# sjtuytc/UnboundedNeRFPytorch

Hardware: AMD Instinct MI355X
Metric: Msamples/sec (Mip-360 garden-shaped 1920x1080x256 frame, FourierGrid render) (higher is better)
Workload: dtype f32; 1 GPU; S1 1920x1080x256 G200 F3(P7) C12 rgbnet 39-128-128-3 f32 stepsize 1.31 thres 1e-4 white-noise grids; rays=2073600, samples_per_ray=256, chunks_per_frame=1, parallelism=1 GPU, step=ray generation + march + shade + un-tiling to image order; 3 frames in flight

## Files before the change

### unboundednerfpytorch_amd/csrc/ugrid_march.hip

```cpp
#include "ugrid_render.h"
#include "ugrid_rays.h"
#include "ugrid_tensorf.h"

__global__ void k_pack_bricks(const float *__restrict__ grid, int P, int C, int X, int Y, int Z, int H,
                              int CH, int coef, float *__restrict__ out, int64_t total) {
  for (int64_t o = (int64_t)blockIdx.x * blockDim.x + threadIdx.x; o < total;
       o += (int64_t)gridDim.x * blockDim.x) {
    int64_t q = o;
    int ch, c;
    if (H == 2) {
      const int qi = (int)(q % (8 * CH)); q /= (8 * CH);
      c = (qi >> 1) & 7;
      ch = (qi >> 4) * 2 + (qi & 1);
    } else {
      ch = (int)(q % CH); q /= CH;
      c = (int)(q % 8); q /= 8;
    }
    const int h = (int)(q % H); q /= H;
    const int k = (int)(q % (Z - 1)); q /= (Z - 1);
    const int j = (int)(q % (Y - 1)); q /= (Y - 1);
    const int i = (int)(q % (X - 1)); q /= (X - 1);
    const int l = (int)q;
    const int chan = h * CH + ch;
    float v = 0.f;
// ... 905 lines not shown
  if (n_rays <= 0) return 0;
  if (n_steps < 2 || !act_shift || mpi_depth < 1 || mpi_depth > 256 || !scratch_w || !scratch_T || !count2 || !alphainv_last)
    return (int)hipErrorInvalidValue;
  ug_train_vox v;
  const int rc = ug_fill_train_vox(&v, mask, mask_dims3, xyz2ijk_scale3, xyz2ijk_shift3);
  if (rc) return rc;
  v.plane_shift = act_shift; v.D = mpi_depth;
  ug_train_args a;
  a.n_rays = n_rays; a.S = n_steps; a.P = 1; a.F = 0; a.X = X; a.Y = Y; a.Z = Z; a.norm_l2 = 0;
  a.cx = a.cy = a.cz = 0.f; a.rx = a.ry = a.rz = 1.f; a.B = 1.f; a.A = 0.f;
  a.shift = 0.f; a.interval = interval; a.thres = thres;
  hipLaunchKernelGGL(HIP_KERNEL_NAME(k_train_march_vox<3>), dim3(ug_blocks(n_rays * UG_WAVE, 256)), dim3(256), 0, ST(s), a, v, density_grid,
                     rays_o, rays_d, (const float *)nullptr, xyz_min, xyz_max, scratch_pts, scratch_density, scratch_step, count, scratch_w,
                     scratch_T, count2, alphainv_last);
  UG_LAUNCH_CHECK();
  return 0;
}

extern "C" int ugrid_train_sample_compact_vox(int64_t n_rays, int32_t slots_per_ray, float act_shift, float interval, float thres,
                                              const float *scratch_pts, const float *scratch_density, const int32_t *scratch_step,
                                              const float *scratch_w, const float *scratch_T, const int32_t *count,
                                              const int64_t *offset_end, const int32_t *count2, const int64_t *offset_end2,
                                              const float *t_table, float *pts1, float *density1, float *weights1, float *T1,
                                              int32_t *pos2, float *pts2, float *density2, float *alpha2, float *weights2,
                                              int64_t *ray_id2, int64_t *step_id2, float *t2, uint8_t *inner2, ugrid_stream_t s) {
  if (n_rays <= 0) return 0;
  hipLaunchKernelGGL(k_train_compact2, dim3(ug_blocks(n_rays * UG_WAVE, 256)), dim3(256), 0, ST(s), n_rays, slots_per_ray, act_shift,
                     interval, thres, scratch_pts, scratch_density, scratch_step, scratch_w, scratch_T, count, offset_end, count2,
                     offset_end2, t_table, pts1, density1, weights1, T1, pos2, pts2, density2, alpha2, weights2, ray_id2, step_id2, t2,
                     inner2, ug_tl_devn.cap > 0 ? ug_tl_devn.cap : INT64_MAX);
  UG_LAUNCH_CHECK();
  return 0;
}

extern "C" int ugrid_train_sample_backward(int64_t n_rays, float act_shift, float interval, const float *density1,
                                           const float *weights1, const float *T1, const int32_t *pos2, const int32_t *count,
                                           const int64_t *offset_end, const float *alphainv_last, const float *g_weights2,
                                           const float *g_alphainv_last, const float *g_density2, float *g_density1,
                                           ugrid_stream_t s) {
  if (n_rays <= 0) return 0;
  hipLaunchKernelGGL(k_train_sample_bwd, dim3(ug_blocks(n_rays * UG_WAVE, 256)), dim3(256), 0, ST(s), n_rays, act_shift, interval,
                     density1, weights1, T1, pos2, count, offset_end, alphainv_last, g_weights2, g_alphainv_last, g_density2, g_density1);
  UG_LAUNCH_CHECK();
  return 0;
}

extern "C" int ugrid_train_compact(int64_t n_rays, int32_t n_samples, const float *scratch_pts, const float *scratch_density,
                                   const int32_t *scratch_step, const int32_t *count, const int64_t *offset_end,
                                   const float *t_table, float *pts, float *density, int64_t *ray_id, int64_t *step_id,
                                   float *t, ugrid_stream_t s) {
  if (n_rays <= 0) return 0;
  hipLaunchKernelGGL(k_train_compact, dim3(ug_blocks(n_rays * UG_WAVE, 256)), dim3(256), 0, ST(s), n_rays, n_samples,
                     scratch_pts, scratch_density, scratch_step, count, offset_end, t_table, pts, density, ray_id, step_id, t);
  UG_LAUNCH_CHECK();
  return 0;
}

template <class MarchTile>
__device__ __forceinline__ void ug_march_block(const ug_ws_view &ws, int64_t nblocks, MarchTile march) {
  const int64_t blk = ug_xcd_remap(blockIdx.x, nblocks);
  if (blk >= nblocks) return;
  const int64_t tile = blk * 4 + (threadIdx.x >> 6);
  if (tile >= ws.n_tiles) return;
  const int n = march(tile, ws.ent + tile * ws.cap, ws.slot + tile * ws.cap);
  if (ug_lane() == 0) ws.count[tile] = n;
}

struct ug_march_geom { ug_ws_view ws; int64_t nblocks; dim3 grid; };
static inline ug_march_geom ug_march_geometry(void *ws_mem, int64_t n_rays, int32_t S) {
  ug_march_geom g;
  g.ws = ug_ws_make(ws_mem, n_rays, S);
  g.nblocks = (g.ws.n_tiles + 3) / 4;
  g.grid = dim3((unsigned)(((g.nblocks + 7) / 8) * 8));
  return g;
}

template <int F, bool L2, int W>
__global__ void __launch_bounds__(256, W)
k_march(ug_march_args a, const float *__restrict__ rays_o, const float *__restrict__ rays_d,
        const float *__restrict__ t_table, const float *__restrict__ s_table,
        const float *__restrict__ bricks, float *__restrict__ alphainv_last, float *__restrict__ depth,
        ug_ws_view ws, int64_t nblocks) {
  ug_march_block(ws, nblocks, [&](int64_t tile, float4 *ent, uint8_t *slot) {
    return ug_march_tile<F, L2>(a, rays_o, rays_d, t_table, s_table, bricks, alphainv_last, depth, tile, ent, slot);
  });
}


template <bool L2>
__global__ void __launch_bounds__(256, 5)
k_march_dcvgo(ug_march_args a, ug_dc_args dc, const float *__restrict__ rays_o, const float *__restrict__ rays_d,
              const float *__restrict__ t_table, const float *__restrict__ s_table, const float *__restrict__ bricks,
              float *__restrict__ alphainv_last, float *__restrict__ depth, float *__restrict__ wsum_mid, ug_ws_view ws,
              int64_t nblocks) {
  ug_march_block(ws, nblocks, [&](int64_t tile, float4 *ent, uint8_t *slot) {
    return ug_march_tile<0, L2, true>(a, rays_o, rays_d, t_table, s_table, bricks, alphainv_last, depth, tile, ent, slot, dc, wsum_mid);
  });
}

__global__ void __launch_bounds__(256, 6)
k_march_dvgo(ug_march_args a, ug_dv_args dv, const float *__restrict__ rays_o, const float *__restrict__ rays_d,
             const float *__restrict__ bricks, float *__restrict__ alphainv_last, float *__restrict__ depth, ug_ws_view ws,
             int64_t nblocks) {
  ug_march_block(ws, nblocks, [&](int64_t tile, float4 *ent, uint8_t *slot) {
    return ug_march_tile_dvgo(a, dv, rays_o, rays_d, bricks, alphainv_last, depth, tile, ent, slot, a.S);
  });
}

__global__ void __launch_bounds__(256, 6)
k_march_mpi(ug_march_args a, ug_mpi_args mp, const float *__restrict__ rays_o, const float *__restrict__ rays_d,
            const float *__restrict__ bricks, const float *__restrict__ act_shift, float *__restrict__ alphainv_last,
            float *__restrict__ depth, ug_ws_view ws, int64_t nblocks) {
  __shared__ float shift[256];
  if ((int)threadIdx.x < mp.D) shift[threadIdx.x] = act_shift[threadIdx.x];
  __syncthreads();
  ug_march_block(ws, nblocks, [&](int64_t tile, float4 *ent, uint8_t *slot) {
    return ug_march_tile_mpi(a, mp, rays_o, rays_d, bricks, shift, alphainv_last, depth, tile, ent, slot);
  });
}

extern "C" int64_t ugrid_render_ws_bytes(int64_t n_rays, int32_t S) {
  const int64_t n_tiles = (n_rays + UG_WAVE - 1) / UG_WAVE, cap = (int64_t)UG_WAVE * S;
  return 256 + ug_align256(n_tiles * 4) + ug_align256(n_tiles * cap * 16) + ug_align256(n_tiles * cap);
}

static int ug_grid_query_any(bool cl, const float *grid, int P, int C, int X, int Y, int Z, const float *xyz,
                             const float *xyz_min, const float *xyz_max, int freq_num, int64_t n, float *out, hipStream_t st) {
  if (n <= 0) return 0;
  if (P != (freq_num > 0 ? 2 * freq_num + 1 : 1)) return (int)hipErrorInvalidValue;
  const int64_t nl = ug_launch_rows(n);
  if (cl)
    hipLaunchKernelGGL(HIP_KERNEL_NAME(k_grid_query<true>), dim3(ug_blocks(nl * C, 256)), dim3(256), 0, st, grid, P, C, X, Y, Z, xyz,
                       xyz_min, xyz_max, freq_num, n, out, ug_tl_devn.ptr);
  else
    hipLaunchKernelGGL(HIP_KERNEL_NAME(k_grid_query<false>), dim3(ug_blocks(nl, 256)), dim3(256), 0, st, grid, P, C, X, Y, Z, xyz,
                       xyz_min, xyz_max, freq_num, n, out, ug_tl_devn.ptr);
  UG_LAUNCH_CHECK();
  return 0;
}

extern "C" int ugrid_grid_query(const float *grid, int P, int C, int X, int Y, int Z, const float *xyz,
                                const float *xyz_min, const float *xyz_max, int freq_num, int64_t n,
                                float *out, ugrid_stream_t s) {
  return ug_grid_query_any(false, grid, P, C, X, Y, Z, xyz, xyz_min, xyz_max, freq_num, n, out, ST(s));
}

extern "C" int ugrid_grid_query_cl(const float *grid, int P, int C, int X, int Y, int Z, const float *xyz,
                                   const float *xyz_min, const float *xyz_max, int freq_num, int64_t n,
                                   float *out, ugrid_stream_t s) {
  return ug_grid_query_any(true, grid, P, C, X, Y, Z, xyz, xyz_min, xyz_max, freq_num, n, out, ST(s));
}

static int ug_grid_query_backward_any(bool cl, const float *grad_out, int P, int C, int X, int Y, int Z, const float *xyz,
                                      const float *xyz_min, const float *xyz_max, int freq_num, int64_t n,
                                      float *grad_grid, hipStream_t st, uint32_t *touch = nullptr) {
  if (n <= 0) return 0;
  if (P != (freq_num > 0 ? 2 * freq_num + 1 : 1)) return (int)hipErrorInvalidValue;
  const int64_t nl = ug_launch_rows(n);
  if (cl)
    hipLaunchKernelGGL(HIP_KERNEL_NAME(k_grid_query_backward<true>), dim3(ug_blocks(nl * P * C, 256)), dim3(256), 0, st, grad_out, P, C,
                       X, Y, Z, xyz, xyz_min, xyz_max, freq_num, n, grad_grid, touch, ug_tl_devn.ptr);
  else
    hipLaunchKernelGGL(HIP_KERNEL_NAME(k_grid_query_backward<false>), dim3(ug_blocks(nl * P, 256)), dim3(256), 0, st, grad_out, P, C,
                       X, Y, Z, xyz, xyz_min, xyz_max, freq_num, n, grad_grid, (uint32_t *)nullptr, ug_tl_devn.ptr);
  UG_LAUNCH_CHECK();
  return 0;
}

extern "C" int ugrid_grid_query_backward(const float *grad_out, int P, int C, int X, int Y, int Z, const float *xyz,
                                         const float *xyz_min, const float *xyz_max, int freq_num, int64_t n,
                                         float *grad_grid, ugrid_stream_t s) {
  return ug_grid_query_backward_any(false, grad_out, P, C, X, Y, Z, xyz, xyz_min, xyz_max, freq_num, n, grad_grid, ST(s));
}

extern "C" int ugrid_grid_query_backward_cl(const float *grad_out, int P, int C, int X, int Y, int Z, const float *xyz,
                                            const float *xyz_min, const float *xyz_max, int freq_num, int64_t n,
                                            float *grad_grid, ugrid_stream_t s) {
  return ug_grid_query_backward_any(true, grad_out, P, C, X, Y, Z, xyz, xyz_min, xyz_max, freq_num, n, grad_grid, ST(s));
}

extern "C" int ugrid_grid_query_backward_cl_touch(const float *grad_out, int P, int C, int X, int Y, int Z, const float *xyz,
                                                  const float *xyz_min, const float *xyz_max, int freq_num, int64_t n,
                                                  float *grad_grid, uint32_t *touch, ugrid_stream_t s) {
  return ug_grid_query_backward_any(true, grad_out, P, C, X, Y, Z, xyz, xyz_min, xyz_max, freq_num, n, grad_grid, ST(s), touch);
}

extern "C" int ugrid_count_views_accumulate(const float *rays_o, const float *rays_d, int64_t n_rays, const float *xyz_min,
                                            const float *xyz_max, float near, float far, float stepdist, int32_t n_samples, int X, int Y,
                                            int Z, float *acc, ugrid_stream_t s) {
  if (n_rays <= 0 || n_samples <= 0) return 0;
  if (!rays_o || !rays_d || !xyz_min || !xyz_max || !acc || X < 1 || Y < 1 || Z < 1) return (int)hipErrorInvalidValue;
  hipLaunchKernelGGL(k_count_views_accumulate, dim3(ug_blocks(n_rays, 64)), dim3(64), 0, ST(s), rays_o, rays_d, n_rays, xyz_min, xyz_max,
                     near, far, stepdist, n_samples, X, Y, Z, acc);
  UG_LAUNCH_CHECK();
  return 0;
}

extern "C" int ugrid_count_views_commit(float *acc, float *count, int64_t n, ugrid_stream_t s) {
  if (n <= 0) return 0;
  if (!acc || !count) return (int)hipErrorInvalidValue;
  const int64_t blocks = ug_blocks(n, 256);
  hipLaunchKernelGGL(k_count_views_commit, dim3((unsigned)(blocks < 65536 ? blocks : 65536)), dim3(256), 0, ST(s), acc, count, n);
  UG_LAUNCH_CHECK();
  return 0;
}

static inline int ug_brick_ch(int C, int *H) {
  if (C == 1) { *H = 1; return 1; }
  *H = 2;
  return UG_CH(C);
}

extern "C" int64_t ugrid_brick_bytes(int P, int C, int X, int Y, int Z, int direct) {
  int H, CH = ug_brick_ch(C, &H);
  if (direct) { H = 1; CH = 4; }
  return (int64_t)P * (X - 1) * (Y - 1) * (Z - 1) * H * 8 * CH * (int64_t)sizeof(float);
}

extern "C" int ugrid_pack_bricks(const float *grid, int P, int C, int X, int Y, int Z, int direct,
                                 float *bricks, ugrid_stream_t s) {
  if (X < 2 || Y < 2 || Z < 2 || P < 1 || C < 1) return (int)hipErrorInvalidValue;
  int H, CH = ug_brick_ch(C, &H);
  if (direct) { H = 1; CH = 4; }
  const int64_t total = (int64_t)P * (X - 1) * (Y - 1) * (Z - 1) * H * 8 * CH;
  int64_t blocks = (total + 255) / 256;
  if (blocks > 256 * 64) blocks = 256 * 64;
  if (C == 12 && !direct) {
    if (P > 1 && (int64_t)(X - 1) * (Y - 1) * (Z - 1) * 384 >= ((int64_t)1 << 32)) return (int)hipErrorInvalidValue;
    hipLaunchKernelGGL(k_pack_quad, dim3((unsigned)blocks), dim3(256), 0, ST(s), grid, P, C, X, Y, Z, bricks, total);
    UG_LAUNCH_CHECK();
    return 0;
  }
  int coef = direct ? 0 : 1;
  hipLaunchKernelGGL(k_pack_bricks, dim3((unsigned)blocks), dim3(256), 0, ST(s), grid, P, C, X, Y, Z, H, CH,
                     coef, bricks, total);
  UG_LAUNCH_CHECK();
  return 0;
}

static int g_march_waves = 6;
extern "C" int ug_set_march_waves(int w) { if (w < 4 || w > 6) return 1; g_march_waves = w; return 0; }

template <int F, int W>
static int ug_march_launch_w(const ugrid_render_params *p, const ug_march_args &a, const float *rays_o,
                             const float *rays_d, const float *t_table, const float *s_table,
                             const float *bricks, float *alphainv_last, float *depth, const ug_march_geom &g,
                             hipStream_t st) {
  if (p->norm_l2)
    hipLaunchKernelGGL(HIP_KERNEL_NAME(k_march<F, true, W>), g.grid, dim3(256), 0, st, a, rays_o,
                       rays_d, t_table, s_table, bricks, alphainv_last, depth, g.ws, g.nblocks);
  else
    hipLaunchKernelGGL(HIP_KERNEL_NAME(k_march<F, false, W>), g.grid, dim3(256), 0, st, a, rays_o,
                       rays_d, t_table, s_table, bricks, alphainv_last, depth, g.ws, g.nblocks);
  UG_LAUNCH_CHECK();
  return 0;
}

template <int F>
static int ug_march_launch(const ugrid_render_params *p, const ug_march_args &a, const float *rays_o,
                           const float *rays_d, const float *t_table, const float *s_table,
                           const float *bricks, float *alphainv_last, float *depth, const ug_march_geom &g,
                           hipStream_t st) {
  switch (g_march_waves) {
    case 4: return ug_march_launch_w<F, 4>(p, a, rays_o, rays_d, t_table, s_table, bricks, alphainv_last, depth, g, st);
    case 6: return ug_march_launch_w<F, 6>(p, a, rays_o, rays_d, t_table, s_table, bricks, alphainv_last, depth, g, st);
    default: return ug_march_launch_w<F, 5>(p, a, rays_o, rays_d, t_table, s_table, bricks, alphainv_last, depth, g, st);
  }
}

extern "C" int ugrid_render_march(const ugrid_render_params *p, const float *rays_o, const float *rays_d,
                                  const float *t_table, const float *s_table, const float *density_bricks,
                                  float *alphainv_last, float *depth, void *ws_mem, ugrid_stream_t s) {
  if (p->n_rays <= 0) return 0;
  ug_march_args a;
  const int rc = ug_fill_march_args(p, a);
  if (rc) return rc;
  const ug_march_geom g = ug_march_geometry(ws_mem, p->n_rays, p->n_samples);
  switch (p->freq_num) {
    case 1: return ug_march_launch<1>(p, a, rays_o, rays_d, t_table, s_table, density_bricks, alphainv_last, depth, g, ST(s));
    case 2: return ug_march_launch<2>(p, a, rays_o, rays_d, t_table, s_table, density_bricks, alphainv_last, depth, g, ST(s));
    case 3: return ug_march_launch<3>(p, a, rays_o, rays_d, t_table, s_table, density_bricks, alphainv_last, depth, g, ST(s));
    case 4: return ug_march_launch<4>(p, a, rays_o, rays_d, t_table, s_table, density_bricks, alphainv_last, depth, g, ST(s));
    case 5: return ug_march_launch<5>(p, a, rays_o, rays_d, t_table, s_table, density_bricks, alphainv_last, depth, g, ST(s));
    default: return (int)hipErrorInvalidValue;
  }
}


extern "C" int ugrid_render_march_dcvgo(const ugrid_render_params *p, const ugrid_dcvgo_params *q, const float *rays_o,
                                        const float *rays_d, const float *t_table, const float *s_table,
                                        const float *density_bricks, float *alphainv_last, float *depth, float *wsum_mid,
                                        void *ws_mem, ugrid_stream_t s) {
  if (p->n_rays <= 0) return 0;
  if (p->freq_num != 0 || !q) return (int)hipErrorInvalidValue;
  ug_march_args a;
  ug_dc_args dc;
  int rc = ug_fill_mask_args(dc, q->mask, q->mask_x, q->mask_y, q->mask_z, q->xyz2ijk_scale, q->xyz2ijk_shift);
  if (!rc) rc = ug_fill_march_args(p, a);
  if (rc) return rc;
  dc.dist_thres = q->dist_thres;
  const ug_march_geom g = ug_march_geometry(ws_mem, p->n_rays, p->n_samples);
  if (p->norm_l2)
    hipLaunchKernelGGL(HIP_KERNEL_NAME(k_march_dcvgo<true>), g.grid, dim3(256), 0, ST(s), a, dc, rays_o, rays_d, t_table,
                       s_table, density_bricks, alphainv_last, depth, wsum_mid, g.ws, g.nblocks);
  else
    hipLaunchKernelGGL(HIP_KERNEL_NAME(k_march_dcvgo<false>), g.grid, dim3(256), 0, ST(s), a, dc, rays_o, rays_d, t_table,
                       s_table, density_bricks, alphainv_last, depth, wsum_mid, g.ws, g.nblocks);
  UG_LAUNCH_CHECK();
  return 0;
}


extern "C" int ugrid_render_march_dvgo(const ugrid_render_params *p, const ugrid_dvgo_params *q, const float *rays_o,
                                       const float *rays_d, const float *density_bricks, float *alphainv_last, float *depth,
                                       void *ws_mem, ugrid_stream_t s) {
  if (p->n_rays <= 0) return 0;
  if (p->freq_num != 0 || !q || !(q->stepdist > 0.f)) return (int)hipErrorInvalidValue;
  ug_march_args a;
  ug_dv_args dv;
  int rc = ug_fill_mask_args(dv, q->mask, q->mask_x, q->mask_y, q->mask_z, q->xyz2ijk_scale, q->xyz2ijk_shift);
  if (!rc) rc = ug_fill_march_args(p, a);
  if (rc) return rc;
  dv.near = q->near_clip; dv.far = q->far_clip; dv.stepdist = q->stepdist;
  const ug_march_geom g = ug_march_geometry(ws_mem, p->n_rays, p->n_samples);
  hipLaunchKernelGGL(k_march_dvgo, g.grid, dim3(256), 0, ST(s), a, dv, rays_o, rays_d, density_bricks, alphainv_last,
                     depth, g.ws, g.nblocks);
  UG_LAUNCH_CHECK();
  return 0;
}



extern "C" int ugrid_render_march_mpi(const ugrid_render_params *p, const ugrid_mpi_params *q, const float *rays_o,
                                      const float *rays_d, const float *density_bricks, const float *act_shift, float *alphainv_last,
                                      float *depth, void *ws_mem, ugrid_stream_t s) {
  if (p->n_rays <= 0) return 0;
  if (p->freq_num != 0 || !q || !act_shift) return (int)hipErrorInvalidValue;
  if (q->mpi_depth < 2 || q->mpi_depth > 256 || q->n_steps < 2 || q->n_steps > p->n_samples) return (int)hipErrorInvalidValue;
  ug_march_args a;
  ug_mpi_args mp;
  int rc = ug_fill_mask_args(mp, q->mask, q->mask_x, q->mask_y, q->mask_z, q->xyz2ijk_scale, q->xyz2ijk_shift);
  if (!rc) rc = ug_fill_march_args(p, a);
  if (rc) return rc;
  mp.D = q->mpi_depth; mp.n = q->n_steps;
  const ug_march_geom g = ug_march_geometry(ws_mem, p->n_rays, p->n_samples);
  hipLaunchKernelGGL(k_march_mpi, g.grid, dim3(256), 0, ST(s), a, mp, rays_o, rays_d, density_bricks, act_shift,
                     alphainv_last, depth, g.ws, g.nblocks);
  UG_LAUNCH_CHECK();
// ... 3 lines not shown
```

### unboundednerfpytorch_amd/csrc/ugrid_render.h

```cpp
#pragma once
#include "ugrid_common.h"
#include "ugrid_math.h"
#include <string.h>

#define UG_CH(C) (2 * (((C) + 3) / 4))
#define UG_MAX_F 5


typedef float f32x16 __attribute__((ext_vector_type(16)));

struct ug_vec3 { float x, y, z; };

__device__ __forceinline__ float ug_norm3_torch(float x, float y, float z) {
  return sqrtf(fmaf(z, z, fmaf(y, y, x * x)));
}

template <bool L2>
__device__ __forceinline__ ug_vec3 ug_contract(ug_vec3 p, float B, float A) {
  const float nrm = L2 ? ug_norm3_torch(p.x, p.y, p.z) : fmaxf(fabsf(p.x), fmaxf(fabsf(p.y), fabsf(p.z)));
  if (!(nrm <= 1.0f)) {
    const float sc = B - (1.0f / nrm) * A;
    p.x = p.x / nrm * sc;
    p.y = p.y / nrm * sc;
    p.z = p.z / nrm * sc;
// ... 20 lines not shown
    a.cell = i0; a.wlo = wlo; a.whi = whi;
  }
  return a;
}

struct ug_cellw { int64_t rec; float w[8]; };

__device__ __forceinline__ ug_cellw ug_cell_setup(float ux, float uy, float uz, int X, int Y, int Z,
                                                 int64_t level_base) {
  const ug_axis ax = ug_axis_setup(ux, X), ay = ug_axis_setup(uy, Y), az = ug_axis_setup(uz, Z);
  ug_cellw r;
  r.rec = level_base + ((int64_t)ax.cell * (Y - 1) + ay.cell) * (Z - 1) + az.cell;
  r.w[0] = az.wlo * ay.wlo * ax.wlo;
  r.w[1] = az.whi * ay.wlo * ax.wlo;
  r.w[2] = az.wlo * ay.whi * ax.wlo;
  r.w[3] = az.whi * ay.whi * ax.wlo;
  r.w[4] = az.wlo * ay.wlo * ax.whi;
  r.w[5] = az.whi * ay.wlo * ax.whi;
  r.w[6] = az.wlo * ay.whi * ax.whi;
  r.w[7] = az.whi * ay.whi * ax.whi;
  return r;
}

template <int F>
struct ug_levels { float cx[2 * F + 1], cy[2 * F + 1], cz[2 * F + 1]; };

template <int F>
__device__ __forceinline__ ug_levels<F> ug_pe(float ux, float uy, float uz) {
  ug_levels<F> L;
  L.cx[0] = ux; L.cy[0] = uy; L.cz[0] = uz;
#pragma unroll
  for (int k = 0; k < F; ++k) {
    const float f = (float)(1 << k);
    float s, c;
    sincosf(f * ux, &s, &c); L.cx[2 * k + 1] = s; L.cx[2 * k + 2] = c;
    sincosf(f * uy, &s, &c); L.cy[2 * k + 1] = s; L.cy[2 * k + 2] = c;
    sincosf(f * uz, &s, &c); L.cz[2 * k + 1] = s; L.cz[2 * k + 2] = c;
  }
  return L;
}

__device__ __forceinline__ float ug_unorm(float p, float lo, float hi) {
  return ((p - lo) / (hi - lo)) * 2.f - 1.f;
}

struct ug_ws_view {
  int32_t *count;
  float4 *ent;
  uint8_t *slot;
  int64_t n_tiles, cap;
};
#define UG_FEAT_STRIDE 12

__host__ __device__ static inline int64_t ug_align256(int64_t x) { return (x + 255) & ~(int64_t)255; }

static inline ug_ws_view ug_ws_make(void *ws, int64_t n_rays, int32_t S) {
  ug_ws_view v;
  v.n_tiles = (n_rays + UG_WAVE - 1) / UG_WAVE;
  v.cap = (int64_t)UG_WAVE * S;
  char *b = (char *)ws + 256;
  v.count = (int32_t *)b;
  b += ug_align256(v.n_tiles * (int64_t)sizeof(int32_t));
  v.ent = (float4 *)b;
  b += ug_align256(v.n_tiles * v.cap * (int64_t)sizeof(float4));
  v.slot = (uint8_t *)b;
  return v;
}

__device__ __forceinline__ int64_t ug_xcd_remap(int64_t b, int64_t nblocks) {
  const int64_t per = (nblocks + 7) / 8;
  return (b % 8) * per + b / 8;
}

struct ug_march_args {
  int64_t n_rays;
  int32_t S, X, Y, Z;
  float cx, cy, cz, rx, ry, rz;
  float lox, loy, loz, hix, hiy, hiz;
  float ex, ey, ez, irx, iry, irz;
  float B, A;
  float shift, interval, thres;
};

__device__ __forceinline__ float ug_density_level(const char *__restrict__ lvl, float cx, float cy, float cz,
                                                  int X, int Y, int Z) {
  const ug_axis_fast ax = ug_axis_inrange(cx, X), ay = ug_axis_inrange(cy, Y), az = ug_axis_inrange(cz, Z);
  const unsigned row = (unsigned)fmaf(ax.cellf, (float)(Y - 1), ay.cellf);
  const unsigned off = __umul24(row, (unsigned)(Z - 1) << 5) + ((unsigned)az.cell << 5);
  const float4 *b = (const float4 *)(lvl + off);
  const float4 v0 = b[0], v1 = b[1];
  const float tz = az.whi, ty = ay.whi, tx = ax.whi;
  const float p00 = fmaf(v0.y, tz, v0.x), p01 = fmaf(v0.w, tz, v0.z);
  const float p10 = fmaf(v1.y, tz, v1.x), p11 = fmaf(v1.w, tz, v1.z);
  return fmaf(fmaf(p11, ty, p10), tx, fmaf(p01, ty, p00));
}

__device__ __forceinline__ void ug_normalise(const ug_march_args &a, float px, float py, float pz, float &ux, float &uy, float &uz) {
  ux = ug_div_r(px - a.lox, a.ex, a.irx) * 2.f - 1.f;
  uy = ug_div_r(py - a.loy, a.ey, a.iry) * 2.f - 1.f;
  uz = ug_div_r(pz - a.loz, a.ez, a.irz) * 2.f - 1.f;
}

__device__ __forceinline__ bool ug_outside_box(const ug_march_args &a, float px, float py, float pz) {
  return (a.lox > px) | (a.loy > py) | (a.loz > pz) | (a.hix < px) | (a.hiy < py) | (a.hiz < pz);
}

struct ug_mask_args {
  const uint8_t *mask;
  int32_t mi, mj, mk;
  float sx, sy, sz, hx, hy, hz;
};

__device__ __forceinline__ bool ug_mask_lookup(const ug_mask_args &m, float px, float py, float pz) {
  float fi = roundf(px * m.sx + m.hx), fj = roundf(py * m.sy + m.hy), fk = roundf(pz * m.sz + m.hz);
  fi = (fi != fi) ? 0.f : fi; fj = (fj != fj) ? 0.f : fj; fk = (fk != fk) ? 0.f : fk;
  if (fi >= 0.f && fi < (float)m.mi && fj >= 0.f && fj < (float)m.mj && fk >= 0.f && fk < (float)m.mk)
    return m.mask[((int64_t)fi * m.mj + (int64_t)fj) * m.mk + (int64_t)fk] != 0;
  return false;
}

static inline int ug_fill_mask_args(ug_mask_args &m, const uint8_t *mask, int32_t mask_x, int32_t mask_y, int32_t mask_z,
                                    const float *scale3, const float *shift3) {
  if (!mask || !scale3 || !shift3 || mask_x < 1 || mask_y < 1 || mask_z < 1) return (int)hipErrorInvalidValue;
  m.mask = mask; m.mi = mask_x; m.mj = mask_y; m.mk = mask_z;
  m.sx = scale3[0]; m.sy = scale3[1]; m.sz = scale3[2];
  m.hx = shift3[0]; m.hy = shift3[1]; m.hz = shift3[2];
  return 0;
}

__device__ __forceinline__ bool ug_composite(float alpha, float thres, float &T, float &w, bool &done) {
  if (!(alpha > thres)) return false;
  w = T * alpha;
  T = (float)((double)T * (1. - (double)alpha));
  if ((double)T < 1e-3) done = true;
  return w > thres;
}

__device__ __forceinline__ void ug_append_survivors(bool surv, float px, float py, float pz, float w, int lane,
                                                    float4 *__restrict__ ent, uint8_t *__restrict__ slot, int &nsurv) {
  const unsigned long long m = __ballot(surv);
  if (m != 0ull) {
    if (surv) {
      const int idx = nsurv + __builtin_amdgcn_mbcnt_hi((unsigned)(m >> 32), __builtin_amdgcn_mbcnt_lo((unsigned)m, 0u));
      ent[idx] = make_float4(px, py, pz, w);
      slot[idx] = (uint8_t)lane;
    }
    nsurv += __popcll(m);
  }
}

struct ug_dc_args : ug_mask_args {
  float dist_thres;
};

template <int F, bool L2, bool DC = false>
__device__ __forceinline__ int ug_march_tile(const ug_march_args &a, const float *__restrict__ rays_o,
                                             const float *__restrict__ rays_d, const float *__restrict__ t_table,
                                             const float *__restrict__ s_table, const float *__restrict__ bricks,
                                             float *__restrict__ alphainv_last, float *__restrict__ depth,
                                             int64_t tile, float4 *__restrict__ ent, uint8_t *__restrict__ slot,
                                             const ug_dc_args &dc = ug_dc_args{}, float *__restrict__ wsum_mid = nullptr) {
  constexpr int P = 2 * F + 1;
  const int lane = ug_lane();
  const int64_t ray = tile * UG_WAVE + lane;
  const bool valid = ray < a.n_rays;

  float ox = 0.f, oy = 0.f, oz = 0.f, dx = 0.f, dy = 0.f, dz = 1.f;
  if (valid) {
    const float rox = rays_o[3 * ray], roy = rays_o[3 * ray + 1], roz = rays_o[3 * ray + 2];
    const float rdx = rays_d[3 * ray], rdy = rays_d[3 * ray + 1], rdz = rays_d[3 * ray + 2];
    ox = (rox - a.cx) / a.rx; oy = (roy - a.cy) / a.ry; oz = (roz - a.cz) / a.rz;
    const float dn = ug_norm3_torch(rdx, rdy, rdz);
    dx = rdx / dn; dy = rdy / dn; dz = rdz / dn;
  }

  const size_t lvl_bytes = (size_t)(a.X - 1) * (a.Y - 1) * (a.Z - 1) * 32;
  const char *__restrict__ bkb = (const char *)bricks;

  float T = 1.f, dsum = 0.f;
  bool done = !valid;
  int nsurv = 0;
  [[maybe_unused]] float cum = 0.f, ppx = 0.f, ppy = 0.f, ppz = 0.f, wmid = 0.f;

  for (int j = 0; j < a.S; ++j) {
    if (__ballot(!done) == 0ull) break;
    bool surv = false;
    float w = 0.f;
    float px = 0.f, py = 0.f, pz = 0.f;
    if (!done) {
      const float t = t_table[j];
      px = ox + dx * t; py = oy + dy * t; pz = oz + dz * t;
      const float nrm = L2 ? ug_norm3_torch(px, py, pz) : fmaxf(fabsf(px), fmaxf(fabsf(py), fabsf(pz)));
      if (!(nrm <= 1.0f)) {
        const float rn = ug_rcp_refined(nrm);
        const float sc = a.B - rn * a.A;
        px = ug_div_r(px, nrm, rn) * sc;
        py = ug_div_r(py, nrm, rn) * sc;
        pz = ug_div_r(pz, nrm, rn) * sc;
      }
      float ux, uy, uz;
      ug_normalise(a, px, py, pz, ux, uy, uz);
      bool keep = true;
      [[maybe_unused]] bool inner = true;
      if constexpr (DC) {
        inner = nrm <= 1.0f;
        keep = inner;
        if (j > 0) {
          cum += ug_norm3_torch(px - ppx, py - ppy, pz - ppz);
          const bool over = cum > dc.dist_thres;
          cum *= over ? 0.f : 1.f;
          keep = keep || over;
        }
        ppx = px; ppy = py; ppz = pz;
        if (keep) keep = ug_mask_lookup(dc, px, py, pz);
      }
      if (keep) {
        float dens = ug_density_level(bkb, ux, uy, uz, a.X, a.Y, a.Z);
#pragma unroll
        for (int k = 0; k < F; ++k) {
          const float f = (float)(1 << k);
          float sx, cx_, sy, cy_, sz, cz_;
          if (k == 0) {
            ug_sincos_small(ux, &sx, &cx_);
            ug_sincos_small(uy, &sy, &cy_);
            ug_sincos_small(uz, &sz, &cz_);
          } else {
            ug_sincos(f * ux, &sx, &cx_);
            ug_sincos(f * uy, &sy, &cy_);
            ug_sincos(f * uz, &sz, &cz_);
          }
          dens += ug_density_level(bkb + (size_t)(2 * k + 1) * lvl_bytes, sx, sy, sz, a.X, a.Y, a.Z);
          dens += ug_density_level(bkb + (size_t)(2 * k + 2) * lvl_bytes, cx_, cy_, cz_, a.X, a.Y, a.Z);
        }
        dens = ug_div_r(dens, (float)P, 1.0f / (float)P);
        const float xs = dens + a.shift;
        const float alpha = ug_alpha(xs, a.interval);
        if (alpha > a.thres) {
          w = T * alpha;
          T = (float)((double)T * (1. - (double)alpha));
          if (w > a.thres) {
            surv = true;
            dsum += w * s_table[j];
            if constexpr (DC) { if (inner) wmid += w; }
          }
          if ((double)T < 1e-3) done = true;
        }
      }
    }
    ug_append_survivors(surv, px, py, pz, w, lane, ent, slot, nsurv);
  }
  if (valid) {
    alphainv_last[ray] = T;
    depth[ray] = dsum;
    if constexpr (DC) wsum_mid[ray] = wmid;
  }
  return nsurv;
}

struct ug_dv_args : ug_mask_args {
  float near, far, stepdist;
};

__device__ __forceinline__ int ug_march_tile_dvgo(const ug_march_args &a, const ug_dv_args &dv, const float *__restrict__ rays_o,
                                                  const float *__restrict__ rays_d, const float *__restrict__ bricks,
                                                  float *__restrict__ alphainv_last, float *__restrict__ depth, int64_t tile,
                                                  float4 *__restrict__ ent, uint8_t *__restrict__ slot, int cap) {
  const int lane = ug_lane();
  const int64_t ray = tile * UG_WAVE + lane;
  const bool valid = ray < a.n_rays;
  float sx = 0.f, sy = 0.f, sz = 0.f, dx = 0.f, dy = 0.f, dz = 0.f;
  int n = 0;
  if (valid) {
    const float ox = rays_o[3 * ray], oy = rays_o[3 * ray + 1], oz = rays_o[3 * ray + 2];
    const float rx = rays_d[3 * ray], ry = rays_d[3 * ray + 1], rz = rays_d[3 * ray + 2];
    const float vx = (rx == 0.f) ? (float)1e-6 : rx, vy = (ry == 0.f) ? (float)1e-6 : ry, vz = (rz == 0.f) ? (float)1e-6 : rz;
    const float ax = (a.hix - ox) / vx, ay = (a.hiy - oy) / vy, az = (a.hiz - oz) / vz;
    const float bx = (a.lox - ox) / vx, by = (a.loy - oy) / vy, bz = (a.loz - oz) / vz;
    const float tmin = fmaxf(fminf(fmaxf(fmaxf(fminf(ax, bx), fminf(ay, by)), fminf(az, bz)), dv.far), dv.near);
    const float tmax = fmaxf(fminf(fminf(fminf(fmaxf(ax, bx), fmaxf(ay, by)), fmaxf(az, bz)), dv.far), dv.near);
    const float rn = sqrtf(rx * rx + ry * ry + rz * rz);
    const double c = (double)ceilf((tmax - tmin) * rn / dv.stepdist);
    const double nn = c > 1. ? c : 1.;
    n = nn > (double)cap ? cap : (int)nn;
    sx = ox + rx * tmin; sy = oy + ry * tmin; sz = oz + rz * tmin;
    dx = rx / rn; dy = ry / rn; dz = rz / rn;
  }
  const char *__restrict__ bkb = (const char *)bricks;
  float T = 1.f, dsum = 0.f;
  bool done = !valid;
  int nsurv = 0;
  for (int j = 0;; ++j) {
    done = done || j >= n;
    if (__ballot(!done) == 0ull) break;
    bool surv = false;
    float w = 0.f, px = 0.f, py = 0.f, pz = 0.f;
    if (!done) {
      const float dist = dv.stepdist * (float)j;
      px = sx + dx * dist; py = sy + dy * dist; pz = sz + dz * dist;
      if (!ug_outside_box(a, px, py, pz) && ug_mask_lookup(dv, px, py, pz)) {
        float ux, uy, uz;
        ug_normalise(a, px, py, pz, ux, uy, uz);
        const float dens = ug_density_level(bkb, ux, uy, uz, a.X, a.Y, a.Z);
        surv = ug_composite(ug_alpha(dens + a.shift, a.interval), a.thres, T, w, done);
        if (surv) dsum += w * (float)j;
      }
    }
    ug_append_survivors(surv, px, py, pz, w, lane, ent, slot, nsurv);
  }
  if (valid) {
    alphainv_last[ray] = T;
    depth[ray] = dsum;
  }
  return nsurv;
}

struct ug_mpi_args : ug_mask_args {
  int32_t D, n;
};

__device__ __forceinline__ int ug_march_tile_mpi(const ug_march_args &a, const ug_mpi_args &mp, const float *__restrict__ rays_o,
                                                 const float *__restrict__ rays_d, const float *__restrict__ bricks,
                                                 const float *__restrict__ shift, float *__restrict__ alphainv_last,
                                                 float *__restrict__ depth, int64_t tile, float4 *__restrict__ ent,
                                                 uint8_t *__restrict__ slot) {
  const int lane = ug_lane();
  const int64_t ray = tile * UG_WAVE + lane;
  const bool valid = ray < a.n_rays;
  float ox = 0.f, oy = 0.f, oz = 0.f, rx = 0.f, ry = 0.f, rz = 0.f;
  if (valid) {
    ox = rays_o[3 * ray]; oy = rays_o[3 * ray + 1]; oz = rays_o[3 * ray + 2];
    rx = rays_d[3 * ray]; ry = rays_d[3 * ray + 1]; rz = rays_d[3 * ray + 2];
  }
// ... 78 lines not shown
}

#ifndef UG_K0_BATCH
#define UG_K0_BATCH 2
#endif

struct ug_shade_args {
  int64_t n_rays;
  int32_t X, Y, Z;
  int32_t residual;
  float lox, loy, loz, hix, hiy, hiz;
  float ex, ey, ez, irx, iry, irz;
};

struct ug_k0_cell { const float4 *rec; float tx, ty, tz; };
template <int CH>
__device__ __forceinline__ ug_k0_cell ug_k0_cell_setup(const float *__restrict__ k0b, int h, int64_t level_base, float cx,
                                                       float cy, float cz, int X, int Y, int Z) {
  const ug_axis_fast ax = ug_axis_inrange(cx, X), ay = ug_axis_inrange(cy, Y), az = ug_axis_inrange(cz, Z);
  const unsigned row = (unsigned)fmaf(ax.cellf, (float)(Y - 1), ay.cellf);
  const unsigned cell = __umul24(row, (unsigned)(Z - 1)) + (unsigned)az.cell;
  ug_k0_cell c;
  c.rec = (const float4 *)(k0b + ((level_base + cell) * 2 + h) * (8 * CH));
  c.tx = ax.whi; c.ty = ay.whi; c.tz = az.whi;
  return c;
}

template <int F, int CH>
__device__ __forceinline__ void ug_k0_gather(const float *__restrict__ k0b, int h, float px, float py, float pz,
                                             const ug_shade_args &a, float (&feat)[CH]) {
  constexpr int P = 2 * F + 1;
  constexpr int NB = UG_K0_BATCH;
  static_assert((8 * CH) % 4 == 0, "half-brick must be a whole number of float4");
  const float ux = ug_div_r(px - a.lox, a.ex, a.irx) * 2.f - 1.f;
  const float uy = ug_div_r(py - a.loy, a.ey, a.iry) * 2.f - 1.f;
  const float uz = ug_div_r(pz - a.loz, a.ez, a.irz) * 2.f - 1.f;
  const int64_t cells = (int64_t)(a.X - 1) * (a.Y - 1) * (a.Z - 1);
  ug_k0_cell c[P];
  c[0] = ug_k0_cell_setup<CH>(k0b, h, 0, ux, uy, uz, a.X, a.Y, a.Z);
#pragma unroll
  for (int k = 0; k < F; ++k) {
    const float f = (float)(1 << k);
    float sx, cx_, sy, cy_, sz, cz_;
    ug_sincos(f * ux, &sx, &cx_);
    ug_sincos(f * uy, &sy, &cy_);
    ug_sincos(f * uz, &sz, &cz_);
    c[2 * k + 1] = ug_k0_cell_setup<CH>(k0b, h, (int64_t)(2 * k + 1) * cells, sx, sy, sz, a.X, a.Y, a.Z);
    c[2 * k + 2] = ug_k0_cell_setup<CH>(k0b, h, (int64_t)(2 * k + 2) * cells, cx_, cy_, cz_, a.X, a.Y, a.Z);
  }
#pragma unroll
  for (int s = 0; s < CH; ++s) feat[s] = 0.f;
#pragma unroll
  for (int b0 = 0; b0 < P; b0 += NB) {
    float4 v[NB][2 * CH];
#pragma unroll
    for (int l = 0; l < NB; ++l)
      if (b0 + l < P) {
#pragma unroll
        for (int q = 0; q < 2 * CH; ++q) v[l][q] = c[b0 + l].rec[q];
      }
    __builtin_amdgcn_sched_barrier(0);
#pragma unroll
    for (int l = 0; l < NB; ++l)
      if (b0 + l < P) {
        const float tz = c[b0 + l].tz, ty = c[b0 + l].ty, tx = c[b0 + l].tx;
#pragma unroll
        for (int pr = 0; pr < CH / 2; ++pr) {
          const float4 q0 = v[l][4 * pr], q1 = v[l][4 * pr + 1], q2 = v[l][4 * pr + 2], q3 = v[l][4 * pr + 3];
          const float a00 = fmaf(q0.z, tz, q0.x), a01 = fmaf(q1.z, tz, q1.x);
          const float a10 = fmaf(q2.z, tz, q2.x), a11 = fmaf(q3.z, tz, q3.x);
          const float b00 = fmaf(q0.w, tz, q0.y), b01 = fmaf(q1.w, tz, q1.y);
          const float b10 = fmaf(q2.w, tz, q2.y), b11 = fmaf(q3.w, tz, q3.y);
          const float fa = fmaf(fmaf(a11, ty, a10), tx, fmaf(a01, ty, a00));
          const float fb = fmaf(fmaf(b11, ty, b10), tx, fmaf(b01, ty, b00));
          feat[2 * pr] = (b0 + l == 0) ? fa : feat[2 * pr] + fa;
          feat[2 * pr + 1] = (b0 + l == 0) ? fb : feat[2 * pr + 1] + fb;
        }
      }
  }
#pragma unroll
  for (int ch = 0; ch < CH; ++ch) feat[ch] = ug_div_r(feat[ch], (float)P, 1.0f / (float)P);
}

typedef float ug_f4 __attribute__((ext_vector_type(4)));
template <int IMM>
__device__ __forceinline__ ug_f4 ug_gload4(unsigned voff, const float *sbase) {
  ug_f4 r;
  asm volatile("global_load_dwordx4 %0, %1, %2 offset:%3" : "=v"(r) : "v"(voff), "s"(sbase), "n"(IMM) : "memory");
  return r;
}
template <int IMM>
__device__ __forceinline__ ug_f4 ug_gload4v(const char *vaddr) {
  ug_f4 r;
  asm volatile("global_load_dwordx4 %0, %1, off offset:%2" : "=v"(r) : "v"(vaddr), "n"(IMM) : "memory");
  return r;
}
template <int N>
__device__ __forceinline__ void ug_vmwait6(ug_f4 (&v)[6]) {
  asm volatile("s_waitcnt vmcnt(%6)" : "+v"(v[0]), "+v"(v[1]), "+v"(v[2]), "+v"(v[3]), "+v"(v[4]), "+v"(v[5]) : "n"(N));
}

template <int K>
__device__ __forceinline__ float ug_quad_bcast(float x) {
  return __int_as_float(__builtin_amdgcn_mov_dpp(__float_as_int(x), K * 0x55, 0xf, 0xf, true));
}

__device__ __forceinline__ void ug_quad_poly(const ug_f4 (&v)[6], float tx, float ty, float tz, bool first, float (&feat)[3]) {
#pragma unroll
  for (int c = 0; c < 3; ++c) {
    const ug_f4 lo = v[2 * c], hi = v[2 * c + 1];
    const float p00 = fmaf(lo.y, tz, lo.x), p01 = fmaf(lo.w, tz, lo.z);
    const float p10 = fmaf(hi.y, tz, hi.x), p11 = fmaf(hi.w, tz, hi.z);
    const float f = fmaf(fmaf(p11, ty, p10), tx, fmaf(p01, ty, p00));
    feat[c] = first ? f : feat[c] + f;
  }
}

struct ug_quad_axis { float lo, ex, ir, nm1, nm2; unsigned goff; };
__device__ __forceinline__ ug_quad_axis ug_quad_axis_of(const ug_shade_args &a, int g) {
  ug_quad_axis q;
  q.lo = g == 0 ? a.lox : (g == 1 ? a.loy : a.loz);
  q.ex = g == 0 ? a.ex : (g == 1 ? a.ey : a.ez);
  q.ir = g == 0 ? a.irx : (g == 1 ? a.iry : a.irz);
  const int n = g == 0 ? a.X : (g == 1 ? a.Y : a.Z);
  q.nm1 = (float)(n - 1); q.nm2 = (float)(n - 2);
  q.goff = (unsigned)g * 16u;
  return q;
}

template <int F, int NBL, int NR>
struct ug_gather_state {
  static constexpr int P = 2 * F + 1, NI = NR * P;
  unsigned off[NI];
  float tx[NI], ty[NI], tz[NI];
  ug_f4 v[NBL][6];
};

#define UG_ISSUE_ITEM(st_, i_)                                                                                     \
  if constexpr (F == 0) {      \
    const char *pa = (const char *)k0b + (uint64_t)st_.off[i_] * 384ull + (uint64_t)((ug_lane() & 3) * 16);        \
    st_.v[(i_) % NBL][0] = ug_gload4v<0>(pa);   st_.v[(i_) % NBL][1] = ug_gload4v<64>(pa);                          \
    st_.v[(i_) % NBL][2] = ug_gload4v<128>(pa); st_.v[(i_) % NBL][3] = ug_gload4v<192>(pa);                         \
    st_.v[(i_) % NBL][4] = ug_gload4v<256>(pa); st_.v[(i_) % NBL][5] = ug_gload4v<320>(pa);                         \
  } else {                                                                                                         \
    const float *lb = k0b + (int64_t)((i_) / NR) * lvl_floats;                                                     \
    st_.v[(i_) % NBL][0] = ug_gload4<0>(st_.off[i_], lb);   st_.v[(i_) % NBL][1] = ug_gload4<64>(st_.off[i_], lb);  \
    st_.v[(i_) % NBL][2] = ug_gload4<128>(st_.off[i_], lb); st_.v[(i_) % NBL][3] = ug_gload4<192>(st_.off[i_], lb); \
    st_.v[(i_) % NBL][4] = ug_gload4<256>(st_.off[i_], lb); st_.v[(i_) % NBL][5] = ug_gload4<320>(st_.off[i_], lb); \
  }

template <int F, int NBL, int NR>
__device__ __forceinline__ void ug_k0_gather_begin(const float *__restrict__ k0b, const ug_shade_args &a,
                                                   const ug_quad_axis &qa, const float (&p_g)[NR],
                                                   ug_gather_state<F, NBL, NR> &st) {
  constexpr int P = 2 * F + 1, NI = NR * P;
#pragma unroll
  for (int r = 0; r < NR; ++r) {
    const float u = ug_div_r(p_g[r] - qa.lo, qa.ex, qa.ir) * 2.f - 1.f;
    float lc[P];
    lc[0] = u;
#pragma unroll
    for (int k = 0; k < F; ++k) {
      if constexpr (F > 0) {
        if (k == 0) ug_sincos_small(u, &lc[1], &lc[2]);
        else ug_sincos((float)(1 << k) * u, &lc[2 * k + 1], &lc[2 * k + 2]);
      }
    }
#pragma unroll
    for (int l = 0; l < P; ++l) {
      const int i = l * NR + r;
      const float ix = fmaf(lc[l], 0.5f, 0.5f) * qa.nm1;
      const float cf = __builtin_amdgcn_fmed3f(floorf(ix), 0.0f, qa.nm2);
      const float wh = ix - cf;
      const float cxf = ug_quad_bcast<0>(cf), cyf = ug_quad_bcast<1>(cf), czf = ug_quad_bcast<2>(cf);
      st.tx[i] = ug_quad_bcast<0>(wh); st.ty[i] = ug_quad_bcast<1>(wh); st.tz[i] = ug_quad_bcast<2>(wh);
      const unsigned row = (unsigned)fmaf(cxf, (float)(a.Y - 1), cyf);
      const unsigned cell = __umul24(row, (unsigned)(a.Z - 1)) + (unsigned)czf;
      if constexpr (F == 0) st.off[i] = cell;
      else st.off[i] = __umul24(cell, 384u) + qa.goff;
    }
  }
  const int64_t lvl_floats = (int64_t)(a.X - 1) * (a.Y - 1) * (a.Z - 1) * 96;
  __builtin_amdgcn_sched_barrier(0);
#pragma unroll
// ... 880 lines not shown
```

Before: 65270 Msamples/s.

## Add software-pipelined ring of level loads in march kernel at 7-8 waves

Adds a ring-buffered density lookup that issues the brick loads for up to three Fourier levels ahead, using explicit vmcnt waits and sched barriers so memory latency overlaps with interpolation math. The march kernel gains 7 and 8 waves-per-SIMD variants, with 8 as the new default. Tile indices are made wave-uniform so the tile base stays scalar, and the t/s tables are read through the constant address space. The cost is more live registers per thread under tighter occupancy limits, which may cause spills, and hand-written inline asm waits that must match the real number of outstanding loads.

```diff
diff --git a/unboundednerfpytorch_amd/csrc/ugrid_march.hip b/unboundednerfpytorch_amd/csrc/ugrid_march.hip
--- a/unboundednerfpytorch_amd/csrc/ugrid_march.hip
+++ b/unboundednerfpytorch_amd/csrc/ugrid_march.hip
@@ -1011,7 +1011,27 @@
         const float *__restrict__ bricks, float *__restrict__ alphainv_last, float *__restrict__ depth,
         ug_ws_view ws, int64_t nblocks) {
   ug_march_block(ws, nblocks, [&](int64_t tile, float4 *ent, uint8_t *slot) {
-    return ug_march_tile<F, L2>(a, rays_o, rays_d, t_table, s_table, bricks, alphainv_last, depth, tile, ent, slot);
+    if constexpr (ug_march_ring<W>::value) {
+      tile = ug_wave_uniform(tile);
+      ent = ws.ent + tile * ws.cap;
+      slot = ws.slot + tile * ws.cap;
+    }
+    return ug_march_tile<F, L2, false, W>(a, rays_o, rays_d, t_table, s_table, bricks, alphainv_last, depth, tile, ent, slot);
+  });
+}
+
+template <int F, bool L2, int W>
+__global__ void __launch_bounds__(256, W)
+k_march_ring(ug_march_args a, const float *__restrict__ rays_o, const float *__restrict__ rays_d,
+             const float *__restrict__ t_table, const float *__restrict__ s_table,
+             const float *__restrict__ bricks, float *__restrict__ alphainv_last, float *__restrict__ depth,
+             ug_ws_view ws, int64_t nblocks) {
+  static_assert(W == 7 || W == 8, "the ring is built for 7 and 8 waves per SIMD");
+  ug_march_block(ws, nblocks, [&](int64_t tile, float4 *ent, uint8_t *slot) {
+    tile = ug_wave_uniform(tile);
+    ent = ws.ent + tile * ws.cap;
+    slot = ws.slot + tile * ws.cap;
+    return ug_march_tile<F, L2, false, W>(a, rays_o, rays_d, t_table, s_table, bricks, alphainv_last, depth, tile, ent, slot);
   });
 }
 
@@ -1167,20 +1187,35 @@
   return 0;
 }
 
-static int g_march_waves = 6;
-extern "C" int ug_set_march_waves(int w) { if (w < 4 || w > 6) return 1; g_march_waves = w; return 0; }
+#define UG_MARCH_WAVES_DEFAULT 8
+static int g_march_waves = UG_MARCH_WAVES_DEFAULT;
+extern "C" int ug_set_march_waves(int w) {
+  if (w == 0) w = UG_MARCH_WAVES_DEFAULT;
+  if (w < 4 || w > 8) return 1;
+  g_march_waves = w;
+  return 0;
+}
 
 template <int F, int W>
 static int ug_march_launch_w(const ugrid_render_params *p, const ug_march_args &a, const float *rays_o,
                              const float *rays_d, const float *t_table, const float *s_table,
                              const float *bricks, float *alphainv_last, float *depth, const ug_march_geom &g,
                              hipStream_t st) {
-  if (p->norm_l2)
-    hipLaunchKernelGGL(HIP_KERNEL_NAME(k_march<F, true, W>), g.grid, dim3(256), 0, st, a, rays_o,
-                       rays_d, t_table, s_table, bricks, alphainv_last, depth, g.ws, g.nblocks);
-  else
-    hipLaunchKernelGGL(HIP_KERNEL_NAME(k_march<F, false, W>), g.grid, dim3(256), 0, st, a, rays_o,
-                       rays_d, t_table, s_table, bricks, alphainv_last, depth, g.ws, g.nblocks);
+  if constexpr (W >= 7) {
+    if (p->norm_l2)
+      hipLaunchKernelGGL(HIP_KERNEL_NAME(k_march_ring<F, true, W>), g.grid, dim3(256), 0, st, a, rays_o,
+                         rays_d, t_table, s_table, bricks, alphainv_last, depth, g.ws, g.nblocks);
+    else
+      hipLaunchKernelGGL(HIP_KERNEL_NAME(k_march_ring<F, false, W>), g.grid, dim3(256), 0, st, a, rays_o,
+                         rays_d, t_table, s_table, bricks, alphainv_last, depth, g.ws, g.nblocks);
+  } else {
+    if (p->norm_l2)
+      hipLaunchKernelGGL(HIP_KERNEL_NAME(k_march<F, true, W>), g.grid, dim3(256), 0, st, a, rays_o,
+                         rays_d, t_table, s_table, bricks, alphainv_last, depth, g.ws, g.nblocks);
+    else
+      hipLaunchKernelGGL(HIP_KERNEL_NAME(k_march<F, false, W>), g.grid, dim3(256), 0, st, a, rays_o,
+                         rays_d, t_table, s_table, bricks, alphainv_last, depth, g.ws, g.nblocks);
+  }
   UG_LAUNCH_CHECK();
   return 0;
 }
@@ -1193,6 +1228,8 @@
   switch (g_march_waves) {
     case 4: return ug_march_launch_w<F, 4>(p, a, rays_o, rays_d, t_table, s_table, bricks, alphainv_last, depth, g, st);
     case 6: return ug_march_launch_w<F, 6>(p, a, rays_o, rays_d, t_table, s_table, bricks, alphainv_last, depth, g, st);
+    case 7: return ug_march_launch_w<F, 7>(p, a, rays_o, rays_d, t_table, s_table, bricks, alphainv_last, depth, g, st);
+    case 8: return ug_march_launch_w<F, 8>(p, a, rays_o, rays_d, t_table, s_table, bricks, alphainv_last, depth, g, st);
     default: return ug_march_launch_w<F, 5>(p, a, rays_o, rays_d, t_table, s_table, bricks, alphainv_last, depth, g, st);
   }
 }
diff --git a/unboundednerfpytorch_amd/csrc/ugrid_render.h b/unboundednerfpytorch_amd/csrc/ugrid_render.h
--- a/unboundednerfpytorch_amd/csrc/ugrid_render.h
+++ b/unboundednerfpytorch_amd/csrc/ugrid_render.h
@@ -126,6 +126,24 @@
   float shift, interval, thres;
 };
 
+typedef float ug_f4 __attribute__((ext_vector_type(4)));
+template <int IMM>
+__device__ __forceinline__ ug_f4 ug_gload4(unsigned voff, const float *sbase) {
+  ug_f4 r;
+  asm volatile("global_load_dwordx4 %0, %1, %2 offset:%3" : "=v"(r) : "v"(voff), "s"(sbase), "n"(IMM) : "memory");
+  return r;
+}
+template <int IMM>
+__device__ __forceinline__ ug_f4 ug_gload4v(const char *vaddr) {
+  ug_f4 r;
+  asm volatile("global_load_dwordx4 %0, %1, off offset:%2" : "=v"(r) : "v"(vaddr), "n"(IMM) : "memory");
+  return r;
+}
+template <int N>
+__device__ __forceinline__ void ug_vmwait6(ug_f4 (&v)[6]) {
+  asm volatile("s_waitcnt vmcnt(%6)" : "+v"(v[0]), "+v"(v[1]), "+v"(v[2]), "+v"(v[3]), "+v"(v[4]), "+v"(v[5]) : "n"(N));
+}
+
 __device__ __forceinline__ float ug_density_level(const char *__restrict__ lvl, float cx, float cy, float cz,
                                                   int X, int Y, int Z) {
   const ug_axis_fast ax = ug_axis_inrange(cx, X), ay = ug_axis_inrange(cy, Y), az = ug_axis_inrange(cz, Z);
@@ -139,6 +157,114 @@
   return fmaf(fmaf(p11, ty, p10), tx, fmaf(p01, ty, p00));
 }
 
+struct ug_ring_setup { unsigned off; float tx, ty, tz; };
+
+__device__ __forceinline__ ug_ring_setup ug_ring_cell(float cx, float cy, float cz, int X, int Y, int Z) {
+  const ug_axis_fast ax = ug_axis_inrange(cx, X), ay = ug_axis_inrange(cy, Y), az = ug_axis_inrange(cz, Z);
+  const unsigned row = (unsigned)fmaf(ax.cellf, (float)(Y - 1), ay.cellf);
+  ug_ring_setup r;
+  r.off = __umul24(row, (unsigned)(Z - 1) << 5) + ((unsigned)az.cell << 5);
+  r.tx = ax.whi; r.ty = ay.whi; r.tz = az.whi;
+  return r;
+}
+
+template <int IMM>
+__device__ __forceinline__ ug_f4 ug_gload4_ro(unsigned voff, const float *sbase) {
+  ug_f4 r;
+  asm volatile("global_load_dwordx4 %0, %1, %2 offset:%3" : "=v"(r) : "v"(voff), "s"(sbase), "n"(IMM));
+  return r;
+}
+
+__device__ __forceinline__ void ug_vmwait2(ug_f4 (&v)[2], int n_after) {
+  if (n_after == 0) asm volatile("s_waitcnt vmcnt(0)" : "+v"(v[0]), "+v"(v[1]));
+  else if (n_after == 1) asm volatile("s_waitcnt vmcnt(2)" : "+v"(v[0]), "+v"(v[1]));
+  else if (n_after == 2) asm volatile("s_waitcnt vmcnt(4)" : "+v"(v[0]), "+v"(v[1]));
+  else if (n_after == 3) asm volatile("s_waitcnt vmcnt(6)" : "+v"(v[0]), "+v"(v[1]));
+  else asm volatile("s_waitcnt vmcnt(8)" : "+v"(v[0]), "+v"(v[1]));
+}
+
+__device__ __forceinline__ int64_t ug_wave_uniform(int64_t x) {
+  const unsigned lo = __builtin_amdgcn_readfirstlane((unsigned)x), hi = __builtin_amdgcn_readfirstlane((unsigned)((uint64_t)x >> 32));
+  return (int64_t)(((uint64_t)hi << 32) | lo);
+}
+
+__device__ __forceinline__ int ug_lane_again() {
+  int zero;
+  asm volatile("s_mov_b32 %0, 0" : "=s"(zero));
+  return __builtin_amdgcn_mbcnt_hi(~0u, __builtin_amdgcn_mbcnt_lo(~0u, (unsigned)zero));
+}
+
+__device__ __forceinline__ float ug_const_ld(const float *__restrict__ table, int j) {
+  return ((const __attribute__((address_space(4))) float *)table)[j];
+}
+
+template <int F, int NFL>
+__device__ __forceinline__ float ug_density_ring(const char *__restrict__ bkb, size_t lvl_bytes, float ux, float uy, float uz,
+                                                 int X, int Y, int Z) {
+  constexpr int P = 2 * F + 1;
+  static_assert(NFL >= 1 && NFL <= 5, "ug_vmwait2 counts up to 4 levels after the one waited for");
+  ug_ring_setup c[NFL];
+  ug_f4 v[NFL][2];
+  float qx = 0.f, qy = 0.f, qz = 0.f;
+#define UG_RING_SETUP(l_)                                                                                              \
+  {                                                                                                                    \
+    if ((l_) == 0) c[0] = ug_ring_cell(ux, uy, uz, X, Y, Z);                                                           \
+    else if (((l_) & 1) == 0) c[(l_) % NFL] = ug_ring_cell(qx, qy, qz, X, Y, Z);                                       \
+    else {                                                                                                             \
+      float sx, sy, sz;                                                                                                \
+      if ((l_) == 1) {               \
+        ug_sincos_small(ux, &sx, &qx); ug_sincos_small(uy, &sy, &qy); ug_sincos_small(uz, &sz, &qz);                   \
+      } else {                                                                                                         \
+        const float f = (float)(1 << ((l_) / 2));                                                                      \
+        ug_sincos(f * ux, &sx, &qx); ug_sincos(f * uy, &sy, &qy); ug_sincos(f * uz, &sz, &qz);                         \
+      }                                                                                                                \
+      c[(l_) % NFL] = ug_ring_cell(sx, sy, sz, X, Y, Z);                                                               \
+    }                                                                                                                  \
+  }
+#define UG_RING_ISSUE(l_)                                                                                              \
+  {                                                                                                                    \
+    const float *lb = (const float *)(bkb + (size_t)(l_) * lvl_bytes);                                                 \
+    v[(l_) % NFL][0] = ug_gload4_ro<0>(c[(l_) % NFL].off, lb);                                                         \
+    v[(l_) % NFL][1] = ug_gload4_ro<16>(c[(l_) % NFL].off, lb);                                                        \
+  }
+  __builtin_amdgcn_sched_barrier(0);
+#pragma unroll
+  for (int l = 0; l < NFL && l < P; ++l) {
+    UG_RING_SETUP(l)
+    __builtin_amdgcn_sched_barrier(0);
+    UG_RING_ISSUE(l)
+  }
+  __builtin_amdgcn_sched_barrier(0);
+  float dens = 0.f;
+#pragma unroll
+  for (int i = 0; i < P; ++i) {
+    ug_vmwait2(v[i % NFL], (P - 1 - i) < (NFL - 1) ? (P - 1 - i) : (NFL - 1));
+    const ug_f4 v0 = v[i % NFL][0], v1 = v[i % NFL][1];
+    const float tz = c[i % NFL].tz, ty = c[i % NFL].ty, tx = c[i % NFL].tx;
+    const float p00 = fmaf(v0.y, tz, v0.x), p01 = fmaf(v0.w, tz, v0.z);
+    const float p10 = fmaf(v1.y, tz, v1.x), p11 = fmaf(v1.w, tz, v1.z);
+    const float d = fmaf(fmaf(p11, ty, p10), tx, fmaf(p01, ty, p00));
+    dens = (i == 0) ? d : dens + d;
+    asm volatile("" :: "v"(dens));
+    __builtin_amdgcn_sched_barrier(0);
+    if (i + NFL < P) {
+      UG_RING_SETUP(i + NFL)
+      __builtin_amdgcn_sched_barrier(0);
+      UG_RING_ISSUE(i + NFL)
+      __builtin_amdgcn_sched_barrier(0);
+    }
+  }
+#undef UG_RING_SETUP
+#undef UG_RING_ISSUE
+  return dens;
+}
+
+#ifndef UG_MARCH_RING6
+#define UG_MARCH_RING6 0
+#endif
+template <int W> struct ug_march_nfl { static constexpr int value = W >= 7 ? 3 : UG_MARCH_RING6; };
+template <int W> struct ug_march_ring { static constexpr bool value = W >= 7 || (W == 6 && UG_MARCH_RING6 > 0); };
+
 __device__ __forceinline__ void ug_normalise(const ug_march_args &a, float px, float py, float pz, float &ux, float &uy, float &uz) {
   ux = ug_div_r(px - a.lox, a.ex, a.irx) * 2.f - 1.f;
   uy = ug_div_r(py - a.loy, a.ey, a.iry) * 2.f - 1.f;
@@ -197,7 +323,7 @@
   float dist_thres;
 };
 
-template <int F, bool L2, bool DC = false>
+template <int F, bool L2, bool DC = false, int W = 6>
 __device__ __forceinline__ int ug_march_tile(const ug_march_args &a, const float *__restrict__ rays_o,
                                              const float *__restrict__ rays_d, const float *__restrict__ t_table,
                                              const float *__restrict__ s_table, const float *__restrict__ bricks,
@@ -232,7 +358,8 @@
     float w = 0.f;
     float px = 0.f, py = 0.f, pz = 0.f;
     if (!done) {
-      const float t = t_table[j];
+      float t;
+      if constexpr (ug_march_ring<W>::value) t = ug_const_ld(t_table, j); else t = t_table[j];
       px = ox + dx * t; py = oy + dy * t; pz = oz + dz * t;
       const float nrm = L2 ? ug_norm3_torch(px, py, pz) : fmaxf(fabsf(px), fmaxf(fabsf(py), fabsf(pz)));
       if (!(nrm <= 1.0f)) {
@@ -259,7 +386,11 @@
         if (keep) keep = ug_mask_lookup(dc, px, py, pz);
       }
       if (keep) {
-        float dens = ug_density_level(bkb, ux, uy, uz, a.X, a.Y, a.Z);
+        float dens;
+        if constexpr (ug_march_ring<W>::value) {
+          dens = ug_density_ring<F, ug_march_nfl<W>::value>(bkb, lvl_bytes, ux, uy, uz, a.X, a.Y, a.Z);
+        } else {
+        dens = ug_density_level(bkb, ux, uy, uz, a.X, a.Y, a.Z);
 #pragma unroll
         for (int k = 0; k < F; ++k) {
           const float f = (float)(1 << k);
@@ -276,6 +407,7 @@
           dens += ug_density_level(bkb + (size_t)(2 * k + 1) * lvl_bytes, sx, sy, sz, a.X, a.Y, a.Z);
           dens += ug_density_level(bkb + (size_t)(2 * k + 2) * lvl_bytes, cx_, cy_, cz_, a.X, a.Y, a.Z);
         }
+        }
         dens = ug_div_r(dens, (float)P, 1.0f / (float)P);
         const float xs = dens + a.shift;
         const float alpha = ug_alpha(xs, a.interval);
@@ -284,7 +416,7 @@
           T = (float)((double)T * (1. - (double)alpha));
           if (w > a.thres) {
             surv = true;
-            dsum += w * s_table[j];
+            if constexpr (ug_march_ring<W>::value) dsum += w * ug_const_ld(s_table, j); else dsum += w * s_table[j];
             if constexpr (DC) { if (inner) wmid += w; }
           }
           if ((double)T < 1e-3) done = true;
@@ -292,6 +424,14 @@
       }
     }
     ug_append_survivors(surv, px, py, pz, w, lane, ent, slot, nsurv);
+  }
+  if constexpr (ug_march_ring<W>::value) {
+    const int64_t ray2 = tile * UG_WAVE + ug_lane_again();
+    if (ray2 < a.n_rays) {
+      alphainv_last[ray2] = T;
+      depth[ray2] = dsum;
+    }
+    return nsurv;
   }
   if (valid) {
     alphainv_last[ray] = T;
@@ -536,24 +676,6 @@
   for (int ch = 0; ch < CH; ++ch) feat[ch] = ug_div_r(feat[ch], (float)P, 1.0f / (float)P);
 }
 
-typedef float ug_f4 __attribute__((ext_vector_type(4)));
-template <int IMM>
-__device__ __forceinline__ ug_f4 ug_gload4(unsigned voff, const float *sbase) {
-  ug_f4 r;
-  asm volatile("global_load_dwordx4 %0, %1, %2 offset:%3" : "=v"(r) : "v"(voff), "s"(sbase), "n"(IMM) : "memory");
-  return r;
-}
-template <int IMM>
-__device__ __forceinline__ ug_f4 ug_gload4v(const char *vaddr) {
-  ug_f4 r;
-  asm volatile("global_load_dwordx4 %0, %1, off offset:%2" : "=v"(r) : "v"(vaddr), "n"(IMM) : "memory");
-  return r;
-}
-template <int N>
-__device__ __forceinline__ void ug_vmwait6(ug_f4 (&v)[6]) {
-  asm volatile("s_waitcnt vmcnt(%6)" : "+v"(v[0]), "+v"(v[1]), "+v"(v[2]), "+v"(v[3]), "+v"(v[4]), "+v"(v[5]) : "n"(N));
-}
-
 template <int K>
 __device__ __forceinline__ float ug_quad_bcast(float x) {
   return __int_as_float(__builtin_amdgcn_mov_dpp(__float_as_int(x), K * 0x55, 0xf, 0xf, true));
```

After: 66290 Msamples/s, median of 6. 1.02x the previous value.
